# HBioquant/DiffBindFR

Hardware: AMD Instinct MI355X
Metric: poses_per_sec (higher is better)
Workload: dtype f32

## Files before the change

### diffbindfr_amd/build.py

```python
import os
import subprocess
import sys
from concurrent.futures import ThreadPoolExecutor

HERE = os.path.dirname(os.path.abspath(__file__))
CSRC = os.path.join(HERE, "csrc")
LIB = os.path.join(HERE, "libdbfr.so")
SOURCES = ["api.cpp", "pack.cpp", "so3_host.cpp", "conv.hip", "conv2.hip", "conv2h.hip", "convz.hip", "graph.hip", "heads.hip", "export.hip", "mdn.hip", "probe.hip", "vina.hip", "modes.hip", "posecheck.hip", "xtc.hip", "sites.hip", "interactions.hip", "pocketcheck.hip", "sasa.hip", "apoholo.hip", "hetero.hip", "hydrogens.hip", "decompose.hip", "cavity.hip", "pocketstates.hip", "shapesim.hip"]
FLAGS = ["--offload-arch=gfx950", "-O3", "-std=c++17", "-fPIC", "-Wno-unused-result"]
if os.environ.get("DBFR_BUILD_DEV") == "1":
    FLAGS.append("-DDBFR_DEV_VARIANTS")
FILE_FLAGS = {"conv.hip": ["-ffp-contract=fast", "-fno-slp-vectorize", "-Wno-array-bounds"] + ([f"-DCONV_NB={os.environ['DBFR_BUILD_NB']}"] if "DBFR_BUILD_NB" in os.environ else [])
              + ([f"-DCONV_PRIO={os.environ['DBFR_BUILD_PRIO']}"] if "DBFR_BUILD_PRIO" in os.environ else [])
              + ([f"-DCONV_XPF={os.environ['DBFR_BUILD_XPF']}"] if "DBFR_BUILD_XPF" in os.environ else [])}
FILE_FLAGS["mdn.hip"] = ["-ffp-contract=off"]
FILE_FLAGS["conv2.hip"] = ["-ffp-contract=fast", "-fno-slp-vectorize", "-Wno-array-bounds"]
FILE_FLAGS["conv2h.hip"] = FILE_FLAGS["conv2.hip"] + ["-Rpass-analysis=kernel-resource-usage"]
FILE_FLAGS["convz.hip"] = FILE_FLAGS["conv2h.hip"]
DEFAULT_FP = ["-ffp-contract=off"]
FILE_FLAGS["vina.hip"] = DEFAULT_FP + ["-Rpass-analysis=kernel-resource-usage"]
FILE_FLAGS["modes.hip"] = FILE_FLAGS["vina.hip"]
FILE_FLAGS["posecheck.hip"] = FILE_FLAGS["vina.hip"]
FILE_FLAGS["xtc.hip"] = FILE_FLAGS["vina.hip"]
FILE_FLAGS["sites.hip"] = FILE_FLAGS["vina.hip"]
FILE_FLAGS["interactions.hip"] = FILE_FLAGS["vina.hip"]
FILE_FLAGS["pocketcheck.hip"] = FILE_FLAGS["vina.hip"]
FILE_FLAGS["sasa.hip"] = FILE_FLAGS["vina.hip"]
FILE_FLAGS["apoholo.hip"] = FILE_FLAGS["vina.hip"]
FILE_FLAGS["hetero.hip"] = FILE_FLAGS["vina.hip"]
FILE_FLAGS["hydrogens.hip"] = FILE_FLAGS["vina.hip"]
FILE_FLAGS["decompose.hip"] = FILE_FLAGS["vina.hip"]
FILE_FLAGS["cavity.hip"] = FILE_FLAGS["vina.hip"]
FILE_FLAGS["pocketstates.hip"] = FILE_FLAGS["vina.hip"]
FILE_FLAGS["shapesim.hip"] = FILE_FLAGS["vina.hip"]


def source_hash(dev=False):
    import hashlib
    h = hashlib.sha256()
    files = sorted([os.path.join(CSRC, f) for f in os.listdir(CSRC) if f.endswith((".cpp", ".hip", ".h", ".inc"))])
    files.append(os.path.join(HERE, "..", "include", "dbfr.h"))
    for f in files:
        h.update(os.path.basename(f).encode())
        h.update(open(f, "rb").read())
    if dev:
        h.update(b"DBFR_DEV_VARIANTS")
    return h.hexdigest()[:16]


def check_m0(hipcc, src):
    import re
    import tempfile
    with tempfile.TemporaryDirectory() as tmp:
        out = os.path.join(tmp, "convz.s")
        cmd = [hipcc, "-x", "hip", "-S", "--cuda-device-only", src, "-o", out] + [f for f in FLAGS + FILE_FLAGS["convz.hip"] if not f.startswith("-Rpass")]
        r = subprocess.run(cmd, capture_output=True, text=True)
        if r.returncode != 0:
            raise RuntimeError("hipcc -S failed (m0 check):\n" + r.stderr)
        lines = open(out).read().splitlines()
    ours = re.compile(r"^\s*s_mov_b32 m0, s\d+\s*$")
    bad = []
    for i, l in enumerate(lines):
        code = l.split(";")[0]
        if re.search(r"\bm0\b", code) and not ours.match(code):
            bad.append(f"{i + 1}: {l.strip()}")
        if ours.match(code) and not any("global_load_lds_dword" in x for x in lines[i + 1:i + 4]):
            bad.append(f"{i + 1}: s_mov_b32 m0 without an LDS-DMA load behind it: {l.strip()}")
    if bad:
        raise RuntimeError("convz.hip: the compiler (or an edit) uses m0 outside the LDS-DMA gathers -- the undeclared writes of prefetch_x are no longer safe:\n  " + "\n  ".join(bad[:10]))


# ... 45 lines not shown
```

### diffbindfr_amd/csrc/api.cpp

```cpp
#include <cmath>
#include <cstdio>
#include <cstring>
#include <algorithm>
#include <atomic>
#include <map>

#include "launch.h"
#include "pack.h"

static unsigned long long convz_sc_lanes(const ConvZ& z) {
  unsigned long long m = 0;
  for (int i = 0; i < z.n_io; ++i) m |= 0xfffull << (z.out_off[i] / 4);
  return m;
}
static inline double fused_bytes(int D_in, int D_out) { return 4.0 * (48 + 9 + 3 + 48 + 48 + D_in + D_out); }

#define RT_TABLE static const
#include "residue_tables.inc"
#undef RT_TABLE

static thread_local std::string g_err;
void dbfr_set_error(const std::string& s) { g_err = s; }
static int fail(int code, const std::string& s) { g_err = s; return code; }

// ... 487 lines not shown
    else atexit([] {
      std::vector<unsigned long long> h(8 * C2_TRACE_CAP);
      if (hipDeviceSynchronize() == hipSuccess && hipMemcpy(h.data(), trace_dev, h.size() * 8, hipMemcpyDeviceToHost) == hipSuccess) {
        if (FILE* f = fopen(getenv("DBFR_CONV2_TRACE"), "wb")) { fwrite(h.data(), 8, h.size(), f); fclose(f); }
      }
    });
  }
  if (trace_dev) (void)hipMemsetAsync(trace_dev, 0, 8 * C2_TRACE_CAP * sizeof(unsigned long long), st);
  return trace_dev;
}

struct ConvJob { const ModelConv* c; ConvSite site; };

static void conv_group(dbfr_model* m, const Ws& w, const ConvJob* jobs, int n, bool fallback, hipStream_t st) {
  AccBatch ab; ab.count = 0;
  ab.wide = 0;
  auto acc = [&](const int* ne, double coef, double* dst) { if (ab.count < ACC_BATCH_MAX) { ab.n[ab.count] = ne; ab.coef[ab.count] = coef; ab.dst[ab.count] = dst; ++ab.count; } };
  auto acc64 = [&](const int64_t* s, double coef, double* dst) { if (ab.count < ACC_BATCH_MAX) { ab.wide |= 1ull << ab.count; acc(reinterpret_cast<const int*>(s), coef, dst); } };
  auto acc_algorithm = [&](const ConvJob& j) {
    const ConvW& cw = j.c->w;
    acc(j.site.n_edges, 2.0 * cw.K * ((double)cw.K + cw.W), m->flops_dev);
    acc(j.site.n_edges, 4.0 * (cw.W + cw.D_in + 9) + 16.0, m->flops_dev + 1);
    acc(j.site.n_edges, fused_bytes(cw.D_in, cw.D_out), m->flops_dev + 2);
  };
  auto timed = [&](bool on, auto&& launch) {
    hipEvent_t e0 = nullptr, e1 = nullptr;
    if (on) {
      prof_events(m, &e0, &e1);
      (void)hipEventRecord(e0, st);
    }
    launch();
    if (on) (void)hipEventRecord(e1, st);
  };
  if (!w.conv2 || !jobs[0].c->k144) {
    if (n == 4) {
      ConvArgs c4[4];
      for (int i = 0; i < 4; ++i) c4[i] = conv_args(jobs[i].site, jobs[i].c->w);
      timed(m->profile == 1, [&] { launch_conv_layer(c4, st); });
    } else {
      for (int i = 0; i < n; ++i) timed(m->profile == 1 && jobs[i].c->k144, [&] { launch_conv(conv_args(jobs[i].site, jobs[i].c->w), st); });
    }
    for (int i = 0; i < n && m->profile; ++i)
      if (jobs[i].c->k144) acc_algorithm(jobs[i]);
    launch_acc_batch(ab, st);
    return;
  }
  const bool f16 = m->gemm_split >= DBFR_GEMM_SPLIT_F16 && !fallback, pair = f16 && m->gemm_split == DBFR_GEMM_REDUCE_FIRST;
  Conv2Args a;
  memset(&a, 0, sizeof a);
  a.queue = m->queue;
  ConvZArgs za;
  memset(&za, 0, sizeof za);
  za.executed = m->profile ? m->flops_dev + 3 : nullptr;
  bool useful_pass = false;
  int n_tiles[4];
  for (int i = 0; i < n; ++i) {
    const ModelConv& c = *jobs[i].c;
    n_tiles[i] = !pair ? c.w2.n_tiles : c.has_w2v ? c.w2v.n_tiles : 0;
    if (!pair || n_tiles[i] > 0) a.c[a.n_conv++] = conv2_desc(jobs[i].site, pair ? c.w2v : c.w2);
    if (pair) {
      za.c[za.n_conv++] = convz_desc(jobs[i].site, c.z, c.w.D_out);
      useful_pass |= !jobs[i].site.chunk_segs;
    }
  }
  timed(m->profile == 1, [&] {
    a.trace = conv2_trace(st);
    if (pair) {
      if (a.n_conv) launch_conv2h(a, st);
      launch_convz(za, st, useful_pass);
    }
    else if (f16) launch_conv2h(a, st);
    else launch_conv2(a, st);
  });
  for (int i = 0; i < n && m->profile; ++i) {
    const ConvZ& z = jobs[i].c->z;
    const int* ne = jobs[i].site.n_edges;
    acc_algorithm(jobs[i]);
    const double rows = 16.0 * n_tiles[i];
    const double ex = f16 ? 3.0 * 2.0 * 144 * (144.0 + rows) : 2.0 * 144 * (144.0 + rows);
    if (!pair || n_tiles[i] > 0) acc(ne, ex, m->flops_dev + 3);
    if (!pair) acc(ne, ex, m->flops_dev + 4);
    else if (n_tiles[i] > 0) acc(ne, 3.0 * 2.0 * 144 * rows, m->flops_dev + 4);
    const int D_in = jobs[i].c->w.D_in, D_out = jobs[i].c->w.D_out;
    const double in_bytes = 4.0 * (48 + 9 + 3 + 48 + 48 + D_in);
    if (!pair) acc(ne, fused_bytes(D_in, D_out), m->flops_dev + 5);
    else acc(ne, in_bytes + 1.0 + (n_tiles[i] > 0 ? in_bytes + 4.0 * (D_out - 48 * z.n_io) : 0.0), m->flops_dev + 5);
    if (pair && jobs[i].site.chunk_segs) {
      double ncv = 0.0;
      for (int io = 0; io < z.n_io; ++io) ncv += (double)z.nc_valid[io];
      acc(ne, 6.0 * (144.0 * 144.0 + 145.0 * ncv), m->flops_dev + 4);
      acc64(jobs[i].site.chunk_segs, 6.0 * 145.0 * 48.0 * ncv, m->flops_dev + 4);
      acc64(jobs[i].site.chunk_segs, 4.0 * 48.0 * z.n_io, m->flops_dev + 5);
    }
  }
  launch_acc_batch(ab, st);
}

static int run_score(dbfr_model* m, const dbfr_batch* B, const dbfr_cond* c, const dbfr_scores* out, Ws& w,
                     hipStream_t st, int step = 0) {
  const dbfr_model_cfg& cfg = m->cfg;
  const int G = B->G, NL = B->NL, NA = B->NA;
  launch_time_embed(c->t, G, cfg.emb_scale, w.temb, st);
  GraphArgs ga;
  ga.b = *B; ga.lig_batch = w.lig_batch; ga.atm_batch = w.atm_batch; ga.is_cab = w.is_cab; ga.n_cab = w.n_cab;
  ga.tr_sigma = c->tr_sigma;
  ga.lig_cut2 = cfg.lig_cutoff * cfg.lig_cutoff; ga.atom_cut2 = cfg.atom_cutoff * cfg.atom_cutoff;
// ... 343 lines not shown
    memcpy(names + pos, e.name.c_str(), e.name.size());
    pos += e.name.size();
    names[pos++] = ';';
    offsets[n] = e.offset; bytes[n] = e.bytes;
    ++n;
  }
  names[pos] = 0;
  return n;
}

static const ModelConv* pick_conv(const dbfr_model* m, int layer, int family) {
  if (layer >= 0 && layer < m->cfg.num_conv_layers && family >= 0 && family < 4) return &m->layer[layer][family];
  if (layer == -1) return &m->final_conv;
  if (layer == -2) return &m->tor;
  if (layer == -3 && !m->cfg.no_sc_torsion) return &m->sc;
  return nullptr;
}

static int test_conv_impl(dbfr_model* m, bool conv2, int32_t layer, int32_t family, int32_t n_edges, const int32_t* n_edges_dev,
                          const int32_t* tgt, const int32_t* gth, const float* emb, const float* sh, const float* tab1, int32_t ld1,
                          const int32_t* idx1, const float* tab2, int32_t ld2, const int32_t* idx2, const float* x, int32_t ldx,
                          float* msg, void* hip_stream) {
  if (!m) return fail(DBFR_ERR_ARG, "null model");
  g_launch_err = false;
  const ModelConv* c = pick_conv(m, layer, family);
  if (!c) return fail(DBFR_ERR_ARG, "no such conv");
  hipStream_t st = (hipStream_t)hip_stream;
  ConvJob job = {c, flat_site(n_edges_dev, n_edges, tgt, gth, emb, sh, tab1, ld1, idx1, tab2, ld2, idx2, x, ldx, msg)};
  bool deep = false;
  if (conv2) {
    if (!c->k144) return fail(DBFR_ERR_ARG, "k_conv2 serves the K=144 convs");
    deep = c->w2.f16_depth > f16_depth_ok();
    const bool rf = m->gemm_split == DBFR_GEMM_REDUCE_FIRST && !deep;
    static int* scratch_dev[16] = {nullptr}; static size_t scratch_dev_ints[16] = {0};
    int dev_id = 0;
    HIPCHECK(hipGetDevice(&dev_id));
    if (dev_id < 0 || dev_id >= 16) return fail(DBFR_ERR_ARG, "test hook: device index beyond 15");
    int*& scratch = scratch_dev[dev_id]; size_t& scratch_ints = scratch_dev_ints[dev_id];
    const int span = 2048, n_span = std::max((n_edges + span - 1) / span, 1), ccap = n_edges / 32 + n_edges / CZ_MAXSEG + n_span + 8;
    if (rf) {
      const size_t need = (size_t)n_span + 1 + 2 * (size_t)ccap;
      if (need > scratch_ints) {
        if (scratch) HIPCHECK(hipFree(scratch));
        scratch = nullptr; scratch_ints = 0;
        HIPCHECK(hipMalloc(&scratch, need * sizeof(int)));
        scratch_ints = need;
      }
      launch_flat_chunks(tgt, n_edges_dev, n_edges, span, n_span, scratch, ccap, scratch + n_span + 1, scratch + n_span + 1 + ccap, st);
    }
    ConvSite& site = job.site;
    if (scratch) { site.chunk_es = scratch + n_span + 1; site.chunk_gl = scratch + n_span + 1 + ccap; site.n_chunks = scratch + n_span; }
    site.max_chunks = ccap;
    if (rf) HIPCHECK(hipMemsetAsync(msg, 0, (size_t)n_edges * c->w.D_out * sizeof(float), st));
  }
  Ws w;
  memset(&w, 0, sizeof w);
  w.conv2 = conv2;
  conv_group(m, w, &job, 1, deep, st);
  HIPCHECK(hipGetLastError());
  return take_launch_error();
}

extern "C" int dbfr_test_sde_step(const dbfr_model* m, const dbfr_batch* b, const dbfr_step* step, const dbfr_scores* scores,
                                  const dbfr_noise* z, float* atom14_out, int32_t* err_word_out, void* hip_stream) {
  int rc = check_batch(m, b);
  if (rc) return rc;
  if (!step || !scores || !z || !err_word_out) return fail(DBFR_ERR_ARG, "dbfr_test_sde_step: null argument");
  if (!scores->tr || !scores->rot || !z->z_tr || !z->z_rot || (b->NTOR > 0 && (!scores->tor || !z->z_tor)) ||
      (!m->cfg.no_sc_torsion && b->NSC > 0 && (!scores->sc_tor || !z->z_sc)))
    return fail(DBFR_ERR_ARG, "dbfr_test_sde_step: null score or noise array");
  hipStream_t st = (hipStream_t)hip_stream;
  HIPCHECK(hipMemsetAsync(err_word_out, 0, sizeof(int32_t), st));
  pose_update(m, b, *step, *scores, z->z_tr, z->z_rot, z->z_tor, z->z_sc, nullptr, atom14_out, nullptr, err_word_out, st);
  HIPCHECK(hipGetLastError());
  return DBFR_OK;
}

extern "C" int dbfr_test_chunk_table(const int32_t* tgt, const int32_t* n_edges_dev, int32_t max_edges, int32_t span, int32_t* scratch, int32_t cap,
                                     int32_t* chunk_es, int32_t* chunk_gl, void* hip_stream) {
  if (!tgt || !n_edges_dev || !scratch || !chunk_es || !chunk_gl || span <= 0 || max_edges < 0 || cap <= 0) return fail(DBFR_ERR_ARG, "dbfr_test_chunk_table: bad argument");
  g_launch_err = false;
  const int n_span = std::max((max_edges + span - 1) / span, 1);
  launch_flat_chunks(tgt, n_edges_dev, max_edges, span, n_span, scratch, cap, chunk_es, chunk_gl, (hipStream_t)hip_stream);
  HIPCHECK(hipGetLastError());
  return take_launch_error();
}

extern "C" int dbfr_test_conv(dbfr_model* m, int32_t layer, int32_t family, int32_t n_edges, const int32_t* n_edges_dev,
                              const int32_t* tgt, const int32_t* gth, const float* emb, const float* sh,
                              const float* tab1, int32_t ld1, const int32_t* idx1, const float* tab2, int32_t ld2,
                              const int32_t* idx2, const float* x, int32_t ldx, float* msg, void* hip_stream) {
  return test_conv_impl(m, false, layer, family, n_edges, n_edges_dev, tgt, gth, emb, sh, tab1, ld1, idx1, tab2, ld2, idx2, x, ldx,
                        msg, hip_stream);
}

extern "C" int dbfr_test_conv2(dbfr_model* m, int32_t layer, int32_t family, int32_t n_edges, const int32_t* n_edges_dev,
                               const int32_t* tgt, const int32_t* gth, const float* emb, const float* sh,
                               const float* tab1, int32_t ld1, const int32_t* idx1, const float* tab2, int32_t ld2,
                               const int32_t* idx2, const float* x, int32_t ldx, float* msg, void* hip_stream) {
  return test_conv_impl(m, true, layer, family, n_edges, n_edges_dev, tgt, gth, emb, sh, tab1, ld1, idx1, tab2, ld2, idx2, x, ldx,
                        msg, hip_stream);
}

extern "C" int dbfr_test_reduce_ln2(dbfr_model* m, int32_t layer, int32_t family, const float* msg, const int32_t* row_start, const int32_t* row_cnt,
                                    int32_t n_nodes, const float* old, int32_t d_old, float* out, int32_t mode, const uint8_t* seg_first, void* hip_stream) {
  if (!m) return fail(DBFR_ERR_ARG, "null model");
// ... 130 lines not shown
```

### diffbindfr_amd/csrc/common.h

```cpp
#pragma once
#include <hip/hip_runtime.h>
#include <stdint.h>
#include <string.h>
#include <string>
#include <vector>

#include "../../include/dbfr.h"

#define NS 48
#define NV 12
#define SH_LD 9
#define EMB 32
#define MAXD 168
#define EDGE_CHUNK 64
int dbfr_edge_chunks(int max_na, int max_nl);

typedef float f32x4 __attribute__((ext_vector_type(4)));
typedef float f32x2 __attribute__((ext_vector_type(2)));
typedef _Float16 f16x8 __attribute__((ext_vector_type(8)));
typedef _Float16 f16x4 __attribute__((ext_vector_type(4)));
typedef _Float16 f16x2 __attribute__((ext_vector_type(2)));
typedef unsigned u32x4 __attribute__((ext_vector_type(4)));
typedef unsigned u32x2 __attribute__((ext_vector_type(2)));

// ... 69 lines not shown
  const int* n_edges; int max_edges;
  const int* gth;
  const float* emb;
  const float* sh;
  const float* tab1; int ld1; const int* idx1;
  const float* tab2; int ld2; const int* idx2;
  const float* x; int ldx;
  ConvW2 w;
  float* msg;
};

struct Conv2Args {
  Conv2Desc c[4];
  int n_conv;
  int* queue;
  int run_barrier, no_split;
  int skew;
  unsigned long long* trace;
};
#define C2_TRACE_CAP 4096

#define CZ_NKT 10
#define CZ_MAXCT 12
#define CZ_MAXSEG 4
#define CZ_TILE_BYTES 6144
struct ConvZ {
  int n_io;
  int nct[2];
  int ct0[2];
  int out_off[2];
  int nc_valid[2];
  const uint32_t* cdesc;
  const void* W2z;
  const float* rowinv;
  const void* W1h; int k1;
  const float* W1rinv;
};
struct ConvZDesc {
  const int* n_edges; int max_edges;
  const int* tgt;
  const int* gth;
  const float* emb; const float* sh;
  const float* tab1; int ld1; const int* idx1;
  const float* tab2; int ld2; const int* idx2;
  const float* x; int ldx;
  ConvZ w;
  float* msg; int D_out;
  const int* chunk_es;
  const int* chunk_gl;
  const int* n_chunks;
  int max_chunks;
  const float* xmax;
};
struct ConvZArgs { ConvZDesc c[4]; int n_conv; float* dbg; double* executed; int dbg_sel; };

static inline uint16_t dbfr_bf16_rne(float x) {
  uint32_t u;
  memcpy(&u, &x, 4);
  u += 0x7fffu + ((u >> 16) & 1u);
  return (uint16_t)(u >> 16);
}
static inline float dbfr_bf16_to_f32(uint16_t b) {
  const uint32_t u = (uint32_t)b << 16;
  float f;
  memcpy(&f, &u, 4);
  return f;
}

struct Mlp2 {
  int in, hid, out;
  const float* w0t;
  const float* b0;
  const float* w1t;
  const float* b1;
};

struct EdgeSet {
  int cap;
  int* n_edges;
  int* tgt;
  int* gth;
  int* aux;
  float* dist;
  float* sh;
  float* emb;
  int* row_start;
  int* row_cnt;
  int* g_cnt;
  int* g_base;
  int* chunk0;
  int* gedge0;
  int* chunk_es;
  int* chunk_gl;
  int chunk_cap;
  uint8_t* seg_first;
};

struct ConvArgs {
  const int* n_edges;
  int max_edges;
  const int* tgt;
  const int* gth;
  const float* emb;
  const float* sh;
  float sh_sign;
  const float* tab1; int ld1; const int* idx1;
  const float* tab2; int ld2; const int* idx2;
// ... 20 lines not shown
```

### diffbindfr_amd/csrc/convz.hip

```cpp
#include <cstdio>
#include <cstdlib>
#include <type_traits>

#include "launch.h"

#define CH_TILE_BYTES 9280
#define CH_TAIL_OFF 8192
#define CH_BIAS_OFF 9216

#define CZ_VSTRIDE 2064
#define CZ_CB (8 * CZ_VSTRIDE)
#define CZ_NCB 2
#define CZ_TILE (CZ_NCB * CZ_CB)
#define CZ_KPB 1
#define CZ_BUF (CZ_KPB * CZ_TILE)
#define CZ_ZBYTES (2 * CZ_BUF)
#define CZ_NHL 2
#define CZ_WAVE_FLOATS (32 * 12 + 32 + 32 + 32 + 32 + 32 + CZ_MAXSEG * 16 + 24 * 64 + CZ_NHL * 256)
#ifndef CZ_PRIO
#define CZ_PRIO 1
#endif
#if CZ_PRIO
#define CZ_SETPRIO(x) __builtin_amdgcn_s_setprio(x)
#else
#define CZ_SETPRIO(x)
#endif
#ifndef CZ_FETCH_AT
#define CZ_FETCH_AT 4
#endif
#ifndef CZ_PF_KT
#define CZ_PF_KT 7
#endif
#define CZ_ZSCALE (-20)

__device__ __forceinline__ void cz_split2(float x0, float x1, unsigned& hi, unsigned& lo) {
  const f16x2 h = __builtin_convertvector((f32x2){x0, x1}, f16x2);
  const f16x2 l = __builtin_convertvector((f32x2){x0 - (float)h[0], x1 - (float)h[1]}, f16x2);
  hi = __builtin_bit_cast(unsigned, h);
  lo = __builtin_bit_cast(unsigned, l);
}
__device__ __forceinline__ float cz_wave_max(float v) {
#pragma unroll
  for (int o = 1; o < 64; o <<= 1) v = fmaxf(v, __shfl_xor(v, o));
  return v;
}

__device__ __forceinline__ int cz_lane_here() {
  int l = __builtin_amdgcn_mbcnt_hi(~0u, __builtin_amdgcn_mbcnt_lo(~0u, 0u));
  asm volatile("" : "+v"(l));
  return l;
}

template <int I, int N, typename F>
__device__ __forceinline__ void cz_static_for(F&& f) {
  if constexpr (I < N) { f(std::integral_constant<int, I>{}); cz_static_for<I + 1, N>(f); }
}

template <int NW, int ABL = 0>
__global__ __launch_bounds__(64 * NW, 2) void k_convz(ConvZArgs a) {
  constexpr int KT = 9;
  extern __shared__ __attribute__((aligned(16))) float lds[];
  const int tid = threadIdx.x, lane = tid & 63, wave = __builtin_amdgcn_readfirstlane(tid >> 6);
  const int n = lane & 15, g = lane >> 4;
  char* zb = reinterpret_cast<char*>(lds);
  float* wl = lds + CZ_ZBYTES / 4 + wave * CZ_WAVE_FLOATS;
  float* w_sh = wl;
  float* w_sa = wl + 32 * 12;
  float* w_ua = w_sa + 32;
  int* w_row = reinterpret_cast<int*>(w_ua + 32);
  int* w_seg = w_row + 32;
  int* w_first = w_seg + 32;
  unsigned* w_mask = reinterpret_cast<unsigned*>(w_first + 32);
  float* w_xs = reinterpret_cast<float*>(w_mask + CZ_MAXSEG * 16);
  u32x4* w_hl = reinterpret_cast<u32x4*>(w_xs + 24 * 64);
  int* b_nseg = reinterpret_cast<int*>(lds + CZ_ZBYTES / 4 + NW * CZ_WAVE_FLOATS);
  int* b_col_edge = b_nseg + NW;
  float* b_col_inv = reinterpret_cast<float*>(b_col_edge + 16 * CZ_NCB);
  unsigned* b_cdesc = reinterpret_cast<unsigned*>(b_col_inv + 16 * CZ_NCB);

  int tr_n = 0;
  auto stamp = [&](int tag) {
    if constexpr ((ABL & 128) != 0) {
      if (a.dbg && blockIdx.x == 0 && lane == 0 && tr_n < 1000) {
        unsigned long long* t = reinterpret_cast<unsigned long long*>(a.dbg) + wave * 1024;
        t[tr_n++] = (__builtin_amdgcn_s_memtime() << 8) | (unsigned)tag;
      }
    }
  };
  int nch[4] = {0, 0, 0, 0}, nu[4] = {0, 0, 0, 0};
#pragma unroll
  for (int c = 0; c < 4; ++c)
    if (c < a.n_conv) {
      const ConvZDesc& d = a.c[c];
      nch[c] = min(*d.n_chunks, d.max_chunks);
      nu[c] = (nch[c] + NW - 1) / NW;
    }
  const int N = nu[0] + nu[1] + nu[2] + nu[3];
  for (int unit = blockIdx.x; unit < N; unit += gridDim.x) {
    int c = 0, ul = unit;
    if (ul >= nu[0]) { ul -= nu[0]; c = 1; if (ul >= nu[1]) { ul -= nu[1]; c = 2; if (ul >= nu[2]) { ul -= nu[2]; c = 3; } } }
    const ConvZDesc& d = a.c[c];
    const ConvZ& W = d.w;
    const int E = min(*d.n_edges, d.max_edges);
    unsigned cd_t = 0u;
    if (tid < (W.ct0[W.n_io - 1] + W.nct[W.n_io - 1]) * 16) cd_t = W.cdesc[tid];
    const int ch = ul * NW + wave;
    int es = 0, len = 0, gidx = 0;
    if (ch < nch[c]) {
      es = d.chunk_es[ch];
      const int gl = d.chunk_gl[ch];
      gidx = gl >> 6;
      len = min(min(gl & 63, 32), max(E - es, 0));
    }
    __syncthreads();
    if (unit != (int)blockIdx.x) tr_n = 1000;
    stamp(1);
    const int sl = lane & 31;
    const bool have = len > 0;
    const int e_sl = have ? es + min(sl, len - 1) : 0;
    const int tgt_ld = d.tgt[e_sl], gth_ld = d.gth[e_sl];
    float s_l[9];
    {
      const float* sp = d.sh + (size_t)e_sl * SH_LD;
#pragma unroll
      for (int k = 0; k < 9; ++k) s_l[k] = sp[k];
    }
    const float xmax_g = d.xmax ? d.xmax[gidx] : 0.f;
    int i1_t[2], i2_t[2];
    f32x4 Ba_t[2][9];
#pragma unroll
    for (int et = 0; et < 2; ++et) {
      const int e = have ? es + min(16 * et + n, len - 1) : 0;
      i1_t[et] = d.idx1[e];
      i2_t[et] = d.idx2[e];
      const float* r0 = d.emb + (size_t)e * NS;
#pragma unroll
      for (int s4 = 0; s4 < 3; ++s4) Ba_t[et][s4] = *reinterpret_cast<const f32x4*>(r0 + 16 * s4 + 4 * g);
    }
    const int tgt_l = have ? tgt_ld : 0, gth_l = have ? gth_ld : 0;
    const int tgt_prev = __shfl_up(tgt_l, 1);
    const bool is_first = lane < 32 && sl < len && (sl == 0 || tgt_l != tgt_prev);
    const unsigned long long bal = __ballot(is_first);
    const unsigned firsts = (unsigned)bal;
    const int nseg = min(__popc(firsts), CZ_MAXSEG);
    const int seg_l = (sl < len) ? __popc(firsts & (0xffffffffu >> (31 - sl))) - 1 : -1;
    if (lane < 32) {
      w_row[sl] = gth_l * d.ldx;
      w_seg[sl] = seg_l;
      if (is_first) w_first[seg_l] = sl;
#pragma unroll
      for (int k = 0; k < 9; ++k) w_sh[sl * 12 + k] = have ? s_l[k] : 0.f;
      w_sh[sl * 12 + 9] = w_sh[sl * 12 + 10] = w_sh[sl * 12 + 11] = 0.f;
    }
    if (lane == 0) b_nseg[wave] = nseg;
    if (tid < CZ_MAXCT * 16) b_cdesc[tid] = cd_t;
    float xmx = 0.f, smx = 0.f;
    if (have) {
      if (d.xmax) xmx = xmax_g;
      else {
        const float* xr = d.x + (size_t)gth_l * d.ldx;
        const int d4 = d.ldx >> 2;
        for (int j = lane >> 5; j < d4; j += 2) {
          const f32x4 v = *reinterpret_cast<const f32x4*>(xr + 4 * j);
          xmx = fmaxf(fmaxf(xmx, fmaxf(fabsf(v[0]), fabsf(v[1]))), fmaxf(fabsf(v[2]), fabsf(v[3])));
        }
      }
      if (lane < 32) {
#pragma unroll
// ... 56 lines not shown
          cz_split2(Ba[s4][0] * sa, Ba[s4][1] * sa, hi0, lo0);
          cz_split2(Ba[s4][2] * sa, Ba[s4][3] * sa, hi1, lo1);
          if (s4 < 8) {
            Ah[et][0][s4 >> 1][2 * (s4 & 1)] = hi0; Ah[et][0][s4 >> 1][2 * (s4 & 1) + 1] = hi1;
            Ah[et][1][s4 >> 1][2 * (s4 & 1)] = lo0; Ah[et][1][s4 >> 1][2 * (s4 & 1) + 1] = lo1;
          } else {
            Atc[et] = (u32x4){lo0, lo1, hi0, hi1};
          }
        }
      }
      __builtin_amdgcn_wave_barrier();
      f32x4 sar[2], uar[2];
#pragma unroll
      for (int et = 0; et < 2; ++et) {
        sar[et] = *reinterpret_cast<const f32x4*>(w_sa + 16 * et + 4 * g);
        uar[et] = *reinterpret_cast<const f32x4*>(w_ua + 16 * et + 4 * g);
      }
      float Hf[KT][2][4];
      float hmx = 0.f;
      f32x4 acc[2];
      cz_static_for<0, 5 * KT>([&](auto ic) {
        constexpr int i = decltype(ic)::value, m = i / 5, sx = i % 5;
        if constexpr (i + 2 < 5 * KT) ldF(std::integral_constant<int, (i + 2 < 5 * KT ? i + 2 : 0)>{});
        if constexpr (sx == 0) { acc[0] = (f32x4){0.f, 0.f, 0.f, 0.f}; acc[1] = (f32x4){0.f, 0.f, 0.f, 0.f}; }
        if constexpr (sx < 4) {
          const f16x8 whi = __builtin_bit_cast(f16x8, F[i % 3][0]), wlo = __builtin_bit_cast(f16x8, F[i % 3][1]);
#pragma unroll
          for (int et = 0; et < 2; ++et) {
            acc[et] = __builtin_amdgcn_mfma_f32_16x16x32_f16(__builtin_bit_cast(f16x8, Ah[et][1][sx]), whi, acc[et], 0, 0, 0);
            acc[et] = __builtin_amdgcn_mfma_f32_16x16x32_f16(__builtin_bit_cast(f16x8, Ah[et][0][sx]), wlo, acc[et], 0, 0, 0);
            acc[et] = __builtin_amdgcn_mfma_f32_16x16x32_f16(__builtin_bit_cast(f16x8, Ah[et][0][sx]), whi, acc[et], 0, 0, 0);
          }
        } else {
          const u32x4 wt = F[i % 3][0];
          const f16x8 wf = __builtin_bit_cast(f16x8, wt);
          const f16x8 wh = __builtin_bit_cast(f16x8, (u32x4){wt[0], wt[1], 0u, 0u});
          const float bias = __builtin_bit_cast(float, F[i % 3][1][0]);
          const float w1r = W.W1rinv ? W.W1rinv[16 * m + n] : 1.f;
#pragma unroll
          for (int et = 0; et < 2; ++et) {
            acc[et] = __builtin_amdgcn_mfma_f32_16x16x32_f16(__builtin_bit_cast(f16x8, Atc[et]), wf, acc[et], 0, 0, 0);
            acc[et] = __builtin_amdgcn_mfma_f32_16x16x32_f16(__builtin_bit_cast(f16x8, (u32x4){Atc[et][2], Atc[et][3], 0u, 0u}), wh, acc[et], 0, 0, 0);
          }
#pragma unroll
          for (int et = 0; et < 2; ++et)
#pragma unroll
            for (int q = 0; q < 4; ++q) {
              const float v = fmaxf(acc[et][q] + bias * sar[et][q], 0.f) * (uar[et][q] * w1r);
              Hf[m][et][q] = v;
              hmx = fmaxf(hmx, v);
            }
        }
      });
      if (!(ABL & 128) && a.dbg && unit == 0 && wave == 0) {
        const float k1i = __builtin_amdgcn_ldexpf(1.f, -W.k1);
#pragma unroll
        for (int m = 0; m < KT; ++m)
#pragma unroll
          for (int et = 0; et < 2; ++et)
#pragma unroll
            for (int q = 0; q < 4; ++q) a.dbg[(16 * et + 4 * g + q) * 144 + 16 * m + n] = Hf[m][et][q] * k1i;
      }
      hmx = cz_wave_max(hmx);
      eh = max(hmx > 0.f ? __builtin_amdgcn_frexp_expf(hmx) : W.k1, W.k1);
      eh = min(eh, W.k1 + 100);
      const float sH = __builtin_amdgcn_ldexpf(1.f, 15 - eh);
#pragma unroll
      for (int m = 0; m < KT; ++m) {
        unsigned h0, l0, h1, l1, h2, l2, h3, l3;
        cz_split2(Hf[m][0][0] * sH, Hf[m][0][1] * sH, h0, l0);
        cz_split2(Hf[m][0][2] * sH, Hf[m][0][3] * sH, h1, l1);
        cz_split2(Hf[m][1][0] * sH, Hf[m][1][1] * sH, h2, l2);
        cz_split2(Hf[m][1][2] * sH, Hf[m][1][3] * sH, h3, l3);
        Hh[m][0] = (u32x4){h0, h1, h2, h3};
        if (m < CZ_NHL) w_hl[m * 64 + lane] = (u32x4){l0, l1, l2, l3};
        else Hh[m][1] = (u32x4){l0, l1, l2, l3};
      }
    }
    const int ephi = 15 - eh + W.k1;
    {
      const _Float16 ph = (_Float16)__builtin_amdgcn_ldexpf(1.f, ephi);
      const unsigned short pb = __builtin_bit_cast(unsigned short, ph);
      u32x4 hb = {0u, 0u, 0u, 0u};
      if (n == 0) {
#pragma unroll
        for (int t = 0; t < 8; ++t) {
          const int slot = t < 4 ? 4 * g + t : 16 + 4 * g + (t - 4);
          if (slot < len) hb[t >> 1] |= (unsigned)pb << (16 * (t & 1));
        }
      }
      Hh[KT][0] = hb;
      Hh[KT][1] = (u32x4){0u, 0u, 0u, 0u};
    }
    stamp(3);
    {
      const int j = lane >> 4, gg = (lane >> 2) & 3, r = lane & 3, t0 = 2 * r;
      const int s0 = t0 < 4 ? 4 * gg + t0 : 16 + 4 * gg + (t0 - 4);
      w_mask[lane] = (w_seg[s0] == j ? 0x0000ffffu : 0u) | (w_seg[s0 + 1] == j ? 0xffff0000u : 0u);
    }
    __builtin_amdgcn_wave_barrier();
    __syncthreads();
    int cbase = 0, total = 0;
#pragma unroll
    for (int v = 0; v < NW; ++v) { const int c = b_nseg[v]; if (v < wave) cbase += c; total += c; }
    cbase = __builtin_amdgcn_readfirstlane(cbase); total = __builtin_amdgcn_readfirstlane(total);
    const int nseg_u = __builtin_amdgcn_readfirstlane(nseg);
    const int ncb = (total + 15) >> 4;
    const float col_inv = __builtin_amdgcn_ldexpf(1.f, -CZ_ZSCALE - ey - ephi);
    const float zs = __builtin_amdgcn_ldexpf(1.f, CZ_ZSCALE);
    if (ABL & 32) continue;
    for (int c = tid; c < 16 * CZ_NCB; c += 64 * NW) b_col_edge[c] = -1;
    __syncthreads();
    if (lane < nseg_u) {
      b_col_edge[cbase + lane] = es + w_first[lane];
      b_col_inv[cbase + lane] = col_inv;
    }
    char* za[CZ_MAXSEG];
    {
      char* zw0 = zb + (n & 7) * CZ_VSTRIDE + g * 512 + (n >> 3) * 256;
#pragma unroll
      for (int j = 0; j < CZ_MAXSEG; ++j) {
        const int col = cbase + j;
        za[j] = j < nseg_u ? zw0 + (col >> 4) * CZ_CB + (col & 15) * 16 : zw0 + CZ_CB + 15 * 16;
      }
    }
    long long n_mfma = 2 * KT * 14;
    for (int io = 0; io < W.n_io; ++io) {
      n_mfma += (long long)W.nct[io] * (3LL * CZ_NKT * CZ_MAXSEG + 9LL * ncb * (KT + (wave == 0)));
      f32x4 acc[3][CZ_NCB];
#pragma unroll
      for (int wt = 0; wt < 3; ++wt)
#pragma unroll
        for (int cb = 0; cb < CZ_NCB; ++cb) acc[wt][cb] = (f32x4){0.f, 0.f, 0.f, 0.f};
      const char* wbase = reinterpret_cast<const char*>(W.W2z) + (size_t)lane * 16;
      int gq = W.ct0[io] * CZ_NKT;
      const int gq_last = (W.ct0[io] + W.nct[io]) * CZ_NKT - 1;
      u32x4 Wf[2][3][2];
      auto fetchW = [&](auto par_c, int q, int share) {
        constexpr int par = decltype(par_c)::value;
        if ((ABL & 1) && q != W.ct0[io] * CZ_NKT) return;
        const char* p = wbase + ((size_t)q * 8 + share) * CZ_TILE_BYTES;
#pragma unroll
        for (int wt = 0; wt < 3; ++wt)
#pragma unroll
          for (int pc = 0; pc < 2; ++pc) Wf[par][wt][pc] = *reinterpret_cast<const u32x4*>(p + (wt * 2 + pc) * 1024);
      };
      u32x4 Ym[CZ_MAXSEG][2];
#pragma unroll
      for (int j = 0; j < CZ_MAXSEG; ++j) { Ym[j][0] = (u32x4){0u, 0u, 0u, 0u}; Ym[j][1] = (u32x4){0u, 0u, 0u, 0u}; }
      auto prefetch_x = [&](int ct) {
        if (nseg_u == 0 || (ABL & 16)) return;
        const int lane = __builtin_amdgcn_mbcnt_hi(~0u, __builtin_amdgcn_mbcnt_lo(~0u, 0u)), n = lane & 15, g = lane >> 4;
        const unsigned cd_n = b_cdesc[(W.ct0[io] + ct) * 16 + n];
        const bool vec = (__builtin_amdgcn_readfirstlane(cd_n) >> 12) & 1u;
        const int xo = cd_n & 0xfff;
        const unsigned lds0 = (unsigned)(size_t)(const void __attribute__((address_space(3)))*)w_xs;
#pragma unroll
        for (int t = 0; t < 8; ++t) {
          const float* xp = d.x + w_row[t < 4 ? 4 * g + t : 16 + 4 * g + (t - 4)] + xo;
          asm volatile("s_mov_b32 m0, %0\n\ts_nop 0\n\tglobal_load_lds_dword %1, off" ::"s"(__builtin_amdgcn_readfirstlane(lds0 + t * 256)), "v"(xp) : "memory");
          if (vec) {
            asm volatile("s_mov_b32 m0, %0\n\ts_nop 0\n\tglobal_load_lds_dword %1, off" ::"s"(__builtin_amdgcn_readfirstlane(lds0 + (8 + t) * 256)), "v"(xp + 1) : "memory");
            asm volatile("s_mov_b32 m0, %0\n\ts_nop 0\n\tglobal_load_lds_dword %1, off" ::"s"(__builtin_amdgcn_readfirstlane(lds0 + (16 + t) * 256)), "v"(xp + 2) : "memory");
// ... 143 lines not shown
      auto tile9 = [&](int ct) {
        constexpr int kt = KT;
        fetchW(K0{}, min(gq + 1, gq_last), wave);
        wait_stage(std::integral_constant<int, 6>{});
        if (wave == 0 && !(ABL & 8)) {
          const int lane = cz_lane_here(), n = lane & 15, g = lane >> 4;
          const char* zr = zb + (kt & 1) * CZ_BUF + g * 512 + n * 16;
#pragma unroll
          for (int cb = 0; cb < CZ_NCB; ++cb)
            if (cb < ncb) {
              f32x4 zf[2];
              zf[0] = *reinterpret_cast<const f32x4*>(zr + cb * CZ_CB); zf[1] = *reinterpret_cast<const f32x4*>(zr + cb * CZ_CB + 256);
              u32x4 ph, pl;
              cut(zf, ph, pl, K0{}); cut(zf, ph, pl, K1{}); cut(zf, ph, pl, K2{}); cut(zf, ph, pl, K3{});
              const f16x8 zh = __builtin_bit_cast(f16x8, ph), zl = __builtin_bit_cast(f16x8, pl);
#pragma unroll
              for (int wt = 0; wt < 3; ++wt) {
                acc[wt][cb] = MF(WFR(wt, 0), zl, acc[wt][cb]);
                acc[wt][cb] = MF(WFR(wt, 1), zh, acc[wt][cb]);
                acc[wt][cb] = MF(WFR(wt, 0), zh, acc[wt][cb]);
              }
            }
        }
        if (ct + 1 < W.nct[io]) { finish_Y(ct + 1); stepA(K0{}, K0{}); }
      };
#undef WFR
      prefetch_x(0);
      wait_stage(K0{});
      auto run_tiles = [&](auto ncb_c) {
        fetchW(K0{}, gq, wave);
        finish_Y(0);
        stepA(K0{}, K0{});
        __syncthreads();
        for (int ct = 0; ct < W.nct[io]; ++ct) {
          cz_static_for<0, CZ_NKT>([&](auto kt_c) {
            constexpr int kt = decltype(kt_c)::value;
            stamp(10);
            if constexpr (kt < KT) {
              tile(kt_c, ncb_c);
              if constexpr (kt == CZ_PF_KT) if (ct + 1 < W.nct[io]) prefetch_x(ct + 1);
            } else
              tile9(ct);
            stamp(12);
            ++gq;
            if (!(ABL & 2)) __syncthreads();
            stamp(13);
          });
        }
      };
      if (ncb > 1) run_tiles(K2{}); else run_tiles(K1{});
#undef YM
#undef MF
#undef SL
      float* red = reinterpret_cast<float*>(zb) + wave * (12 * CZ_NCB * 64);
#pragma unroll
      for (int wt = 0; wt < 3; ++wt)
#pragma unroll
        for (int cb = 0; cb < CZ_NCB; ++cb)
#pragma unroll
          for (int q = 0; q < 4; ++q) red[((wt * CZ_NCB + cb) * 4 + q) * 64 + lane] = acc[wt][cb][q];
      __syncthreads();
      for (int idx = tid; idx < 16 * ncb * 48; idx += 64 * NW) {
        const int col = idx / 48, w = idx - 48 * col;
        const int e = b_col_edge[col];
        if (e >= 0) {
          const int r = w & 15;
          const float* rp = reinterpret_cast<const float*>(zb) + (((w >> 4) * CZ_NCB + (col >> 4)) * 4 + (r & 3)) * 64 + 16 * (r >> 2) + (col & 15);
          float s = 0.f;
#pragma unroll
          for (int v = 0; v < NW; ++v) s += rp[v * (12 * CZ_NCB * 64)];
          d.msg[(size_t)e * d.D_out + W.out_off[io] + w] = s * b_col_inv[col] * W.rowinv[io * 48 + w];
        }
      }
      __syncthreads();
    }
    if (a.executed && lane == 0) atomicAdd(a.executed, 16384.0 * (double)n_mfma);
  }
}

__global__ void k_convz_useful(ConvZArgs a) {
  for (int c = 0; c < a.n_conv; ++c) {
    const ConvZDesc& d = a.c[c];
    const ConvZ& W = d.w;
    const int nch = min(*d.n_chunks, d.max_chunks), E = min(*d.n_edges, d.max_edges);
    double useful = 0.0, bytes = 0.0;
    for (int ch = blockIdx.x * blockDim.x + threadIdx.x; ch < nch; ch += gridDim.x * blockDim.x) {
      const int es = d.chunk_es[ch], len = min(min(d.chunk_gl[ch] & 63, 32), max(E - es, 0));
      int nseg = 0;
      for (int i = 0; i < len; ++i) nseg += (i == 0 || d.tgt[es + i] != d.tgt[es + i - 1]);
      nseg = min(nseg, CZ_MAXSEG);
      double u = 144.0 * 144.0 * len;
      for (int io = 0; io < W.n_io; ++io) u += (double)W.nc_valid[io] * 145.0 * ((double)len + 48.0 * nseg);
      useful += 6.0 * u;
      bytes += 4.0 * 48.0 * W.n_io * nseg;
    }
    if (useful > 0.0) { atomicAdd(a.executed + 1, useful); atomicAdd(a.executed + 2, bytes); }
  }
}

size_t convz_lds_bytes() { return CZ_ZBYTES + 8 * CZ_WAVE_FLOATS * sizeof(float) + (8 + 2 * 16 * CZ_NCB + CZ_MAXCT * 16) * sizeof(int); }

void launch_convz(const ConvZArgs& a0, hipStream_t st, bool useful_pass) {
  constexpr int NW = 8;
  ConvZArgs a = a0;
  static float* dbg_dev = nullptr;
  static const char* dbg_file = getenv("DBFR_CONVZ_DEBUG");
  if (dbg_file && !dbg_dev) {
    if (hipMalloc(&dbg_dev, 8 * 1024 * 8) != hipSuccess || hipMemset(dbg_dev, 0, 8 * 1024 * 8) != hipSuccess) dbg_dev = nullptr;
    else atexit([] {
      std::vector<float> h(8 * 1024 * 2);
      if (hipDeviceSynchronize() == hipSuccess && hipMemcpy(h.data(), dbg_dev, h.size() * 4, hipMemcpyDeviceToHost) == hipSuccess)
        if (FILE* f = fopen(getenv("DBFR_CONVZ_DEBUG"), "wb")) { fwrite(h.data(), 4, h.size(), f); fclose(f); }
    });
  }
  a.dbg = dbg_dev;
  const size_t lds = convz_lds_bytes();
#define V(x) { if (dbfr_launch_check(hipFuncSetAttribute(reinterpret_cast<const void*>(&k_convz<NW, x>), hipFuncAttributeMaxDynamicSharedMemorySize, (int)lds), "k_convz: hipFuncSetAttribute(MaxDynamicSharedMemorySize)")) return; \
               hipLaunchKernelGGL((k_convz<NW, x>), dim3(dbfr_current_cu_count()), dim3(64 * NW), lds, st, a); return; }
#ifdef DBFR_DEV_VARIANTS
  static int abl = getenv("DBFR_CONVZ_ABL") ? atoi(getenv("DBFR_CONVZ_ABL")) : 0;
  if (abl == 1) V(1) if (abl == 2) V(2) if (abl == 4) V(4) if (abl == 8) V(8) if (abl == 16) V(16) if (abl == 32) V(32) if (abl == 12) V(12) if (abl == 5) V(5) if (abl == 64) V(64) if (abl == 128) V(128)
#endif
  if (a.executed && useful_pass) hipLaunchKernelGGL(k_convz_useful, dim3(64), dim3(256), 0, st, a);
  V(0)
#undef V
}
```

Measured before the change: 548.2.

## Hand out tail convz work units dynamically via an atomic ticket counter

The convz kernel used to stride statically over work units with blockIdx. It now processes the first rounds statically and then claims the last few rounds of units dynamically through an atomic ticket in global memory, so workgroups that finish early take more work instead of sitting idle at the tail. The ticket is zeroed by a memset before the launch and reset by the last finishing block. It also adds a timing probe variant and turns off the compiler's atomic optimizer for this file. The cost is extra global atomics plus a cross-block reset protocol that has to stay correct.

```diff
diff --git a/diffbindfr_amd/build.py b/diffbindfr_amd/build.py
--- a/diffbindfr_amd/build.py
+++ b/diffbindfr_amd/build.py
@@ -16,7 +16,7 @@
 FILE_FLAGS["mdn.hip"] = ["-ffp-contract=off"]
 FILE_FLAGS["conv2.hip"] = ["-ffp-contract=fast", "-fno-slp-vectorize", "-Wno-array-bounds"]
 FILE_FLAGS["conv2h.hip"] = FILE_FLAGS["conv2.hip"] + ["-Rpass-analysis=kernel-resource-usage"]
-FILE_FLAGS["convz.hip"] = FILE_FLAGS["conv2h.hip"]
+FILE_FLAGS["convz.hip"] = FILE_FLAGS["conv2h.hip"] + ["-mllvm", "-amdgpu-atomic-optimizer-strategy=None"]
 DEFAULT_FP = ["-ffp-contract=off"]
 FILE_FLAGS["vina.hip"] = DEFAULT_FP + ["-Rpass-analysis=kernel-resource-usage"]
 FILE_FLAGS["modes.hip"] = FILE_FLAGS["vina.hip"]
diff --git a/diffbindfr_amd/csrc/api.cpp b/diffbindfr_amd/csrc/api.cpp
--- a/diffbindfr_amd/csrc/api.cpp
+++ b/diffbindfr_amd/csrc/api.cpp
@@ -563,6 +563,7 @@
   ConvZArgs za;
   memset(&za, 0, sizeof za);
   za.executed = m->profile ? m->flops_dev + 3 : nullptr;
+  za.ticket = m->queue + 2;
   bool useful_pass = false;
   int n_tiles[4];
   for (int i = 0; i < n; ++i) {
@@ -1012,6 +1013,7 @@
     if (scratch) { site.chunk_es = scratch + n_span + 1; site.chunk_gl = scratch + n_span + 1 + ccap; site.n_chunks = scratch + n_span; }
     site.max_chunks = ccap;
     if (rf) HIPCHECK(hipMemsetAsync(msg, 0, (size_t)n_edges * c->w.D_out * sizeof(float), st));
+    if (rf) HIPCHECK(hipMemsetAsync(m->queue + 2, 0, 8, st));
   }
   Ws w;
   memset(&w, 0, sizeof w);
diff --git a/diffbindfr_amd/csrc/common.h b/diffbindfr_amd/csrc/common.h
--- a/diffbindfr_amd/csrc/common.h
+++ b/diffbindfr_amd/csrc/common.h
@@ -145,7 +145,7 @@
   int max_chunks;
   const float* xmax;
 };
-struct ConvZArgs { ConvZDesc c[4]; int n_conv; float* dbg; double* executed; int dbg_sel; };
+struct ConvZArgs { ConvZDesc c[4]; int n_conv; float* dbg; double* executed; int dbg_sel; int* ticket; int dyn_rounds; };
 
 static inline uint16_t dbfr_bf16_rne(float x) {
   uint32_t u;
diff --git a/diffbindfr_amd/csrc/convz.hip b/diffbindfr_amd/csrc/convz.hip
--- a/diffbindfr_amd/csrc/convz.hip
+++ b/diffbindfr_amd/csrc/convz.hip
@@ -1,5 +1,7 @@
 #include <cstdio>
+#include <algorithm>
 #include <cstdlib>
+#include <cstring>
 #include <type_traits>
 
 #include "launch.h"
@@ -31,6 +33,11 @@
 #ifndef CZ_PF_KT
 #define CZ_PF_KT 7
 #endif
+#ifndef CZ_DYN_ROUNDS
+#define CZ_DYN_ROUNDS 2
+#endif
+#define CZ_DBG_WG 320
+#define CZ_DBG_LAUNCHES 640
 #define CZ_ZSCALE (-20)
 
 __device__ __forceinline__ void cz_split2(float x0, float x1, unsigned& hi, unsigned& lo) {
@@ -77,6 +84,7 @@
   int* b_col_edge = b_nseg + NW;
   float* b_col_inv = reinterpret_cast<float*>(b_col_edge + 16 * CZ_NCB);
   unsigned* b_cdesc = reinterpret_cast<unsigned*>(b_col_inv + 16 * CZ_NCB);
+  int* b_tick = reinterpret_cast<int*>(b_cdesc + CZ_MAXCT * 16);
 
   int tr_n = 0;
   auto stamp = [&](int tag) {
@@ -96,7 +104,21 @@
       nu[c] = (nch[c] + NW - 1) / NW;
     }
   const int N = nu[0] + nu[1] + nu[2] + nu[3];
-  for (int unit = blockIdx.x; unit < N; unit += gridDim.x) {
+  const bool dyn = !(ABL & 32) && a.dyn_rounds > 0;
+  const int n_static = dyn ? max(0, N / (int)gridDim.x - a.dyn_rounds) * (int)gridDim.x : N;
+  if constexpr ((ABL & 256) != 0) {
+    if (a.dbg && tid == 0) {
+      reinterpret_cast<unsigned long long*>(a.dbg)[(size_t)blockIdx.x * 3] = __builtin_amdgcn_s_memrealtime();
+      b_tick[1] = 0;
+    }
+  }
+  int unit = blockIdx.x;
+  if (dyn && n_static == 0) {
+    if (tid == 0) b_tick[0] = atomicAdd(a.ticket, 1);
+    __syncthreads();
+    unit = __builtin_amdgcn_readfirstlane(b_tick[0]);
+  }
+  while (unit < N) {
     int c = 0, ul = unit;
     if (ul >= nu[0]) { ul -= nu[0]; c = 1; if (ul >= nu[1]) { ul -= nu[1]; c = 2; if (ul >= nu[2]) { ul -= nu[2]; c = 3; } } }
     const ConvZDesc& d = a.c[c];
@@ -114,6 +136,7 @@
     }
     __syncthreads();
     if (unit != (int)blockIdx.x) tr_n = 1000;
+    if constexpr ((ABL & 256) != 0) { if (tid == 0) ++b_tick[1]; }
     stamp(1);
     const int sl = lane & 31;
     const bool have = len > 0;
@@ -276,7 +299,7 @@
             }
         }
       });
-      if (!(ABL & 128) && a.dbg && unit == 0 && wave == 0) {
+      if (!(ABL & (128 | 256)) && a.dbg && unit == 0 && wave == 0) {
         const float k1i = __builtin_amdgcn_ldexpf(1.f, -W.k1);
 #pragma unroll
         for (int m = 0; m < KT; ++m)
@@ -332,7 +355,7 @@
     const int ncb = (total + 15) >> 4;
     const float col_inv = __builtin_amdgcn_ldexpf(1.f, -CZ_ZSCALE - ey - ephi);
     const float zs = __builtin_amdgcn_ldexpf(1.f, CZ_ZSCALE);
-    if (ABL & 32) continue;
+    if (ABL & 32) { unit += gridDim.x; continue; }
     for (int c = tid; c < 16 * CZ_NCB; c += 64 * NW) b_col_edge[c] = -1;
     __syncthreads();
     if (lane < nseg_u) {
@@ -582,6 +605,9 @@
 #undef YM
 #undef MF
 #undef SL
+      int ticket = 0;
+      const bool ask = dyn && io == W.n_io - 1 && unit + (int)gridDim.x >= n_static;
+      if (ask && tid == 0) ticket = atomicAdd(a.ticket, 1);
       float* red = reinterpret_cast<float*>(zb) + wave * (12 * CZ_NCB * 64);
 #pragma unroll
       for (int wt = 0; wt < 3; ++wt)
@@ -602,9 +628,22 @@
           d.msg[(size_t)e * d.D_out + W.out_off[io] + w] = s * b_col_inv[col] * W.rowinv[io * 48 + w];
         }
       }
+      if (ask && tid == 0) b_tick[0] = n_static + ticket;
       __syncthreads();
     }
     if (a.executed && lane == 0) atomicAdd(a.executed, 16384.0 * (double)n_mfma);
+    unit = dyn && unit + (int)gridDim.x >= n_static ? __builtin_amdgcn_readfirstlane(b_tick[0]) : unit + (int)gridDim.x;
+  }
+  if constexpr ((ABL & 256) != 0) {
+    if (a.dbg && tid == 0) {
+      unsigned long long* t = reinterpret_cast<unsigned long long*>(a.dbg) + (size_t)blockIdx.x * 3;
+      t[1] = __builtin_amdgcn_s_memrealtime();
+      t[2] = (unsigned long long)b_tick[1];
+    }
+  }
+  if (dyn && tid == 0) {
+    const int dn = atomicAdd(a.ticket + 1, 1);
+    if (dn == (int)gridDim.x - 1) { a.ticket[0] = 0; a.ticket[1] = 0; __threadfence(); }
   }
 }
 
@@ -628,17 +667,26 @@
   }
 }
 
-size_t convz_lds_bytes() { return CZ_ZBYTES + 8 * CZ_WAVE_FLOATS * sizeof(float) + (8 + 2 * 16 * CZ_NCB + CZ_MAXCT * 16) * sizeof(int); }
+size_t convz_lds_bytes() { return CZ_ZBYTES + 8 * CZ_WAVE_FLOATS * sizeof(float) + (8 + 2 * 16 * CZ_NCB + CZ_MAXCT * 16 + 4) * sizeof(int); }
 
 void launch_convz(const ConvZArgs& a0, hipStream_t st, bool useful_pass) {
   constexpr int NW = 8;
   ConvZArgs a = a0;
+  static const int deal_rounds = [] {
+    const char* e = getenv("DBFR_CONVZ_DEAL");
+    if (!e || !*e) return CZ_DYN_ROUNDS;
+    return strcmp(e, "static") == 0 ? 0 : std::max(atoi(e), 1);
+  }();
+  a.dyn_rounds = a.ticket ? deal_rounds : 0;
+  for (int c = 0; c < a.n_conv; ++c)
+    if (a.c[c].w.n_io < 1) a.dyn_rounds = 0;
   static float* dbg_dev = nullptr;
   static const char* dbg_file = getenv("DBFR_CONVZ_DEBUG");
+  constexpr size_t dbg_head = 8 * 1024 * 8, dbg_launch = (size_t)CZ_DBG_WG * 3 * 8, dbg_bytes = dbg_head + CZ_DBG_LAUNCHES * dbg_launch;
   if (dbg_file && !dbg_dev) {
-    if (hipMalloc(&dbg_dev, 8 * 1024 * 8) != hipSuccess || hipMemset(dbg_dev, 0, 8 * 1024 * 8) != hipSuccess) dbg_dev = nullptr;
+    if (hipMalloc(&dbg_dev, dbg_bytes) != hipSuccess || hipMemset(dbg_dev, 0, dbg_bytes) != hipSuccess) dbg_dev = nullptr;
     else atexit([] {
-      std::vector<float> h(8 * 1024 * 2);
+      std::vector<float> h(dbg_bytes / 4);
       if (hipDeviceSynchronize() == hipSuccess && hipMemcpy(h.data(), dbg_dev, h.size() * 4, hipMemcpyDeviceToHost) == hipSuccess)
         if (FILE* f = fopen(getenv("DBFR_CONVZ_DEBUG"), "wb")) { fwrite(h.data(), 4, h.size(), f); fclose(f); }
     });
@@ -649,6 +697,14 @@
                hipLaunchKernelGGL((k_convz<NW, x>), dim3(dbfr_current_cu_count()), dim3(64 * NW), lds, st, a); return; }
 #ifdef DBFR_DEV_VARIANTS
   static int abl = getenv("DBFR_CONVZ_ABL") ? atoi(getenv("DBFR_CONVZ_ABL")) : 0;
+  if (abl == 256) {
+    static int n_launch = 0;
+    if (dbg_dev && n_launch < CZ_DBG_LAUNCHES && dbfr_current_cu_count() <= CZ_DBG_WG) {
+      a.dbg = reinterpret_cast<float*>(reinterpret_cast<char*>(dbg_dev) + dbg_head + n_launch++ * dbg_launch);
+      V(256)
+    }
+    a.dbg = nullptr;
+  }
   if (abl == 1) V(1) if (abl == 2) V(2) if (abl == 4) V(4) if (abl == 8) V(8) if (abl == 16) V(16) if (abl == 32) V(32) if (abl == 12) V(12) if (abl == 5) V(5) if (abl == 64) V(64) if (abl == 128) V(128)
 #endif
   if (a.executed && useful_pass) hipLaunchKernelGGL(k_convz_useful, dim3(64), dim3(256), 0, st, a);
```

Result: no change. 550.2 (median of 2 runs) (+0.4%).
